# Ego-J/I2VSGG

Measured on AMD Instinct MI355X. Metric: frames/sec (600x1000, 32 ROI/frame), higher is better.
Workload: dtype f32; 1 GPU; BASELINE.json configs[1]: cfgs/res101.yml, SGG_emb fwd+bwd+SGD, 2 frames/GPU 600x1000, 32 boxes + 32 pairs/frame, ResNet-101 C4; frames_per_gpu=2, global_frames=2, hip_graph=True, parallelism=dp1 (frames sharded, RCCL all-reduce of vrd grads)

## Files before the change

### i2vsgg_amd/_lib.py

```python
import ctypes as C
import os

import torch

_HERE = os.path.dirname(os.path.abspath(__file__))
LIB_PATH = os.path.join(_HERE, "libi2vsgg_hip.so")

LAYOUT_NHWC, LAYOUT_NCHW = 0, 1
EPI_RELU, EPI_RESIDUAL, EPI_SCALE, EPI_BIAS, EPI_ZEROED = 1, 2, 4, 8, 16

_p, _i, _f, _z, _l = C.c_void_p, C.c_int32, C.c_float, C.c_size_t, C.c_int64

SIGNATURES = {
    "i2v_version": (_i, []),
    "i2v_last_error": (C.c_char_p, []),
    "i2v_build_flags": (_i, []),
    "i2v_stream_create": (_i, [_i, _i, C.POINTER(C.c_void_p)]),
    "i2v_stream_destroy": (_i, [_p]),
    "i2v_roi_align_fwd": (_i, [_p, _i, _i, _i, _i, _i, _p, _i, _i, _i, _f, _i, _p, _i, _p]),
    "i2v_roi_align_bwd": (_i, [_p, _i, _p, _i, _i, _i, _f, _i, _p, _i, _i, _i, _i, _i, _p]),
    "i2v_roi_align_bwd_gather_workspace_bytes": (_z, [_i, _i, _i, _i, _i]),
    "i2v_roi_align_bwd_gather": (_i, [_p, _p, _i, _i, _i, _f, _i, _p, _i, _i, _i, _i, _p, _z, _p]),
    "i2v_roi_align_sampled_fwd": (_i, [_p, _i, _i, _i, _i, _i, _p, _i, _i, _i, _f, _i, _p, _i, _p]),
    "i2v_roi_align_sampled_bwd": (_i, [_p, _i, _p, _i, _i, _i, _f, _i, _p, _i, _i, _i, _i, _i, _p]),
    "i2v_roi_pool_fwd": (_i, [_p, _i, _i, _i, _i, _i, _p, _i, _i, _i, _f, _p, _p, _i, _p]),
    "i2v_roi_pool_fwd_geom": (_i, [_p, _i, _i, _p, _l, _p, _i, _i, _i, _f, _p, _p, _i, _p]),
    "i2v_roi_pool_bwd": (_i, [_p, _p, _i, _p, _i, _i, _i, _p, _i, _i, _i, _i, _i, _p]),
    "i2v_nms_workspace_bytes": (_z, [_i, _i]),
    "i2v_nms_sorted": (_i, [_p, _i, _i, _f, _i, _p, _p, _p, _z, _p]),
    "i2v_rpn_proposal_workspace_bytes": (_z, [_i, _i, _i, _i, _i]),
    "i2v_rpn_proposal": (_i, [_p, _i, _p, _p, _p, _i, _i, _i, _i, _i, _i, _i, _f, _p, _p, _p, _p, _z, _p]),
    "i2v_rpn_decode": (_i, [_p, _i, _p, _p, _p, _i, _i, _i, _i, _i, _p, _p, _p]),
    "i2v_sort_desc_workspace_bytes": (_z, [_i, _i]),
    "i2v_sort_desc": (_i, [_p, _i, _i, _p, _p, _z, _p]),
    "i2v_bbox_overlaps": (_i, [_p, _i, _i, _i, _p, _i, _i, _i, _p, _p, _p, _p]),
    "i2v_conv_fwd": (_i, [_p, _p, _p, _p, _p, _p, _i, _i, _i, _i, _i, _i, _i, _i, _i, _i, _p, _z, _p]),
    "i2v_conv_fwd_splits": (_i, [_i, _i, _i, _i, _i, _i, _i, _i, _i, _z]),
    "i2v_conv_split_workspace_bytes": (_z, [_i, _i, _i, _i, _i, _i, _i, _i, _i]),
    "i2v_conv_fwd_plan": (_i, [_i, _i, _i, _i, _i, _i, _i, _i, _i, _i, _i, _z, _p, _i]),
    "i2v_conv_wgrad_plan": (_i, [_i, _i, _i, _i, _i, _i, _i, _i, _i, _i, _i, _i, _i, _i, _z, _p, _i]),
    "i2v_set_tuning": (_i, [_i, _i]),
    "i2v_get_tuning": (_i, [_i]),
    "i2v_gemm_nt_batched": (_i, [_p, _p, _p, _i, _i, _i, _i, _l, _l, _l, _p, _z, _p]),
    "i2v_winograd_filter": (_i, [_p, _p, _i, _i, _p]),
    "i2v_conv3x3_winograd_workspace_bytes": (_z, [_i, _i, _i, _i, _i]),
    "i2v_conv3x3_winograd_fwd": (_i, [_p, _p, _p, _p, _p, _i, _i, _i, _i, _i, _i, _p, _z, _p]),
    "i2v_winograd4_filter": (_i, [_p, _p, _i, _i, _p]),
    "i2v_winograd4_filter_dgrad": (_i, [_p, _p, _i, _i, _p]),
    "i2v_conv3x3_winograd4_workspace_bytes": (_z, [_i, _i, _i, _i, _i]),
    "i2v_conv3x3_winograd4_fwd": (_i, [_p, _p, _p, _p, _p, _i, _i, _i, _i, _i, _i, _p, _z, _p]),
    "i2v_conv_set_tile": (_i, [_i]),
    "i2v_conv_debug_clock": (_i, [_p]),
    "i2v_debug_clock_stamp": (_i, [_p, _p]),
    "i2v_conv_dgrad_workspace_bytes": (_z, [_i, _i, _i, _i]),
    "i2v_conv_dgrad": (_i, [_p, _p, _p, _i, _i, _i, _i, _i, _i, _i, _i, _i, _p, _z, _p, _z, _p]),
    "i2v_conv_wgrad_workspace_bytes": (_z, [_i, _i, _i, _i, _i, _i, _i, _i, _i]),
    "i2v_conv_wgrad": (_i, [_p, _p, _p, _i, _i, _i, _i, _i, _i, _i, _i, _i, _f, _p, _z, _p]),
    "i2v_conv_dgrad_fused": (_i, [_p, _p, _p, _p, _p, _p, _p, _i, _i, _i, _i, _i, _i, _i, _i, _i, _p, _z, _p, _z, _p]),
    "i2v_conv_wgrad_scaled": (_i, [_p, _p, _p, _p, _i, _i, _i, _i, _i, _i, _i, _i, _i, _f, _p, _z, _p]),
    "i2v_ordered_fallbacks": (_i, [_i]),
    "i2v_conv3x3_winograd4_dgrad": (_i, [_p, _p, _p, _p, _p, _i, _i, _i, _i, _i, _p, _z, _p]),
    "i2v_conv3x3_winograd4_wgrad_workspace_bytes": (_z, [_i, _i, _i, _i, _i]),
    "i2v_conv3x3_winograd4_wgrad": (_i, [_p, _p, _p, _p, _i, _i, _i, _i, _i, _f, _p, _z, _p]),
    "i2v_gemm_tn_batched": (_i, [_p, _p, _p, _i, _i, _i, _i, _l, _l, _l, _p]),
    "i2v_gemm_tn_batched_acc": (_i, [_p, _p, _p, _i, _i, _i, _i, _l, _l, _l, _p]),
    "i2v_conv3x3_winograd4_v_bytes": (_z, [_i, _i, _i, _i]),
    "i2v_conv3x3_winograd4_fwd_keep": (_i, [_p, _p, _p, _p, _p, _p, _i, _i, _i, _i, _i, _i, _p, _z, _p]),
    "i2v_conv3x3_winograd4_wgrad_v": (_i, [_p, _p, _p, _p, _i, _i, _i, _i, _i, _f, _p, _z, _p]),
    "i2v_conv_wgrad_sgd": (_i, [_p, _p, _p, _p, _i, _i, _i, _i, _i, _i, _i, _i, _i, _f, _f, _f, _p]),
    "i2v_epilogue_bwd": (_i, [_p, _p, _p, _p, _p, _p, _l, _i, _i, _p, _p, _z, _p]),
    "i2v_maxpool3x3s2_fwd": (_i, [_p, _p, _p, _i, _i, _i, _i, _p]),
    "i2v_sgd_momentum": (_i, [_p, _p, _p, _l, _f, _f, _f, _p]),
    "i2v_sgd_momentum_multi": (_i, [_p, _p, _p, _p, _p, _p, _i, _f, _p]),
    "i2v_adam_step": (_i, [_p, _p]),
    "i2v_adam_multi": (_i, [_p, _p, _p, _p, _p, _p, _p, _i, C.c_double, C.c_double, C.c_double, _p, _p]),
    "i2v_dstyle_pool_fwd": (_i, [_p, _p, _p, _l, _i, _i, _i, _p]),
    "i2v_dstyle_pool_bwd": (_i, [_p, _p, _p, _p, _p, _l, _i, _i, _i, _p]),
    "i2v_dstyle_fused_workspace_bytes": (_z, [_l, _i, _i, _i]),
    "i2v_dstyle_fused_fwd": (_i, [_p, _p, _p, _p, _p, _p, _p, _p, _l, _i, _i, _i, _i, _p, _z, _p]),
    "i2v_relation_topk_workspace_bytes": (_z, [_i, _i]),
    "i2v_relation_topk": (_i, [_p, _p, _p, _p, _i, _i, _i, _p, _p, _p, _p, _z, _p]),
    "i2v_video_associate_workspace_bytes": (_z, [_i, _i, _i]),
    "i2v_video_associate": (_i, [_p, _p, _p, _p, _p, _p, _i, _i, _i, _i, _p, _p, _p, _p, _p, _p, _z, _p]),
    "i2v_video_viou_match_workspace_bytes": (_z, [_i, _i]),
    "i2v_video_viou_match": (_i, [_p, _p, _p, _p, _p, _p, _i, _i, _i, _l, _i, _i, C.c_double, _p, _p, _p, _p, _z, _p]),
    "i2v_seqnms_workspace_bytes": (_z, [_i, _i, _i]),
    "i2v_seqnms": (_i, [_p, _p, _p, _p, _p, _i, _i, _i, C.c_double, C.c_double, _i, _p, _p, _p, _p, _z, _p]),
    "i2v_det_eval_match_workspace_bytes": (_z, [_i]),
    "i2v_det_eval_match": (_i, [_p, _p, _p, _p, _p, _p, _p, _i, _i, _i, _i, _i, C.c_double, _p, _p, _p, _p, _z, _p]),
    "i2v_det_eval_curve_workspace_bytes": (_z, [_i]),
    "i2v_det_eval_curve": (_i, [_p, _p, _p, _p, _i, _i, _p, _p, _p, _p, _p, _p, _p, _p, _z, _p]),
    "i2v_image_prep_size": (_i, [_i, _i, _i, _p, _p, _p]),
    "i2v_image_prep": (_i, [_p, _i, _i, _i, _i, _p, _i, _p, _i, _i, _p]),
    "i2v_det_postprocess_workspace_bytes": (_z, [_i, _i]),
    "i2v_det_postprocess": (_i, [_p, _p, _p, _i, _p, _p, _f, _f, _f, _i, _i, _f, _f, _i, _p, _p, _p, _z, _p]),
    "i2v_det_postprocess_info": (_i, [_p, _p, _p, _i, _p, _p, _p, _i, _i, _f, _f, _i, _p, _p, _p, _z, _p]),
    "i2v_l2norm_rows_fwd": (_i, [_p, _p, _p, _i, _i, _f, _p]),
    "i2v_l2norm_rows_bwd": (_i, [_p, _p, _p, _p, _i, _i, _f, _p]),
    "i2v_bce_rows_fwd": (_i, [_p, _p, _p, _p, _i, _i, _p]),
    "i2v_bce_rows_bwd": (_i, [_p, _p, _p, _p, _p, _i, _i, _p]),
    "i2v_half_mse_fwd": (_i, [_p, _l, _f, _p, _p]),
    "i2v_half_mse_bwd": (_i, [_p, _l, _f, _p, _p, _p]),
    "i2v_smooth_l1_fwd": (_i, [_p, _p, _p, _p, _l, _i, _i, _f, _p, _p]),
    "i2v_smooth_l1_bwd": (_i, [_p, _p, _p, _p, _l, _i, _i, _f, _p, _p, _p]),
    "i2v_bbox_transform": (_i, [_p, _i, _p, _i, _p, _i, _i, _p, _p, _p]),
    "i2v_signed_sqrt_fwd": (_i, [_p, _p, _l, _p]),
    "i2v_signed_sqrt_bwd": (_i, [_p, _p, _p, _l, _p]),
    "i2v_pair_gather_fwd": (_i, [_p, _p, _p, _p, _i, _i, _i, _p]),
    "i2v_pair_gather_bwd": (_i, [_p, _p, _p, _p, _i, _i, _i, _p]),
    "i2v_dpixel_fwd": (_i, [_p, _p, _p, _p, _p, _p, _p, _p, _i, _i, _p]),
    "i2v_dpixel_bwd_workspace_bytes": (_z, []),
    "i2v_dpixel_bwd": (_i, [_p, _p, _p, _p, _p, _p, _p, _p, _p, _p, _p, _p, _i, _i, _f, _p, _z, _p]),
}


class I2VError(RuntimeError):
    pass


def _load():
    if not os.path.exists(LIB_PATH):
        raise ImportError(
            "i2vsgg_amd: %s not found. Build it with `python -c 'import __graft_entry__ as g; g.build()'` "
# ... 48 lines not shown
```

### i2vsgg_amd/conv_route.py

```python
from collections import namedtuple

EPI_RELU, EPI_RESIDUAL, EPI_SCALE, EPI_BIAS = 1, 2, 4, 8

DIRECT = "direct"
WINOGRAD = "winograd"
AS_WGRAD = "as_wgrad"
WINOGRAD_X = "winograd_x"
WINOGRAD_V = "winograd_v"
NONE = "none"
ARENA, FRESH = "arena", "fresh"

Switches = namedtuple("Switches", "winograd_train winograd_wgrad winograd_keep_v winograd_train_min_c linear_dgrad_as_wgrad "
                                  "small_gw_bytes")
Route = namedtuple("Route", "fwd keep_v dgrad dgrad_pad transposed_g wgrad flags as_linear")


def whole_filter_as_linear(in_shape, w_shape, pad, has_res):
    _, _, H, W = in_shape
    _, _, KH, KW = w_shape
    return pad == 0 and KH == H and KW == W and (KH > 1 or KW > 1) and not has_res


def epilogue_flags(scale, shift, res, relu):
    return (EPI_SCALE if scale else EPI_BIAS if shift else 0) | (EPI_RESIDUAL if res else 0) | (EPI_RELU if relu else 0)


def plan_dgrad(in_shape, w_shape, stride, pad, sw):
    B, Cin, H, W = in_shape
    Cout, _, KH, KW = w_shape
    if ((H, W, KH, KW, stride, pad) == (1, 1, 1, 1, 1, 0) and B <= Cin
            and (Cout * Cin >= sw.linear_dgrad_as_wgrad or Cout % 4 != 0)):
        return AS_WGRAD, 0
    return DIRECT, (-Cout) % 4


def plan_conv(in_shape, w_shape, stride, pad, sw, scale=False, shift=False, res=False, relu=False, winograd_ok=False,
              needs_x=False, needs_w=False, needs_bias=False, in_block=False):
    as_linear = whole_filter_as_linear(in_shape, w_shape, pad, res)
    if as_linear:
        (B, Cin, H, W), Cout = in_shape, w_shape[0]
        in_shape, w_shape = (B, H * W * Cin, 1, 1), (Cout, H * W * Cin, 1, 1)
    B, Cin, H, W = in_shape
    Cout, _, KH, KW = w_shape
    flags = epilogue_flags(scale, shift, res, relu)
    eligible = (sw.winograd_train and (KH, KW, stride, pad) == (3, 3, 1, 1) and Cin >= sw.winograd_train_min_c
                and Cout >= sw.winograd_train_min_c and Cin % 4 == 0)
    wgrad_ok = eligible and sw.winograd_wgrad and Cout % 4 == 0
    if in_block:
        fwd = WINOGRAD if eligible else DIRECT
        keep_v = bool(eligible and sw.winograd_keep_v and wgrad_ok)
        wgrad = NONE if not needs_w else (WINOGRAD_V if keep_v else WINOGRAD_X) if wgrad_ok else DIRECT
        return Route(fwd, keep_v, fwd, 0, False, wgrad, flags, as_linear)
    fwd_wino = bool(winograd_ok and eligible and (needs_x or needs_w) and not res)
    keep_v = bool(fwd_wino and sw.winograd_keep_v and needs_w and wgrad_ok)
    dgrad_wino = fwd_wino or wgrad_ok
    plain, plain_pad = plan_dgrad(in_shape, w_shape, stride, pad, sw)
    dgrad = NONE if not needs_x else WINOGRAD if dgrad_wino else plain
    transposed_g = bool(dgrad == AS_WGRAD and (relu or scale or needs_bias))
    wgrad = NONE if not needs_w else (WINOGRAD_V if keep_v else WINOGRAD_X) if wgrad_ok else DIRECT
    return Route(WINOGRAD if fwd_wino else DIRECT, keep_v, dgrad, plain_pad if dgrad == DIRECT else 0, transposed_g, wgrad,
                 flags, as_linear)


def wgrad_placement(n_elems, pixels, has_arena, sw):
    return ARENA if has_arena and n_elems * 4 <= sw.small_gw_bytes and pixels > 224 else FRESH
```

### i2vsgg_amd/csrc/api.cpp

```cpp
#include <hip/hip_runtime.h>
#include <stdarg.h>
#include <stdio.h>
#include "../../include/i2vsgg_hip.h"

static thread_local char g_err[512] = "";

void i2v_set_error(const char* fmt, ...) {
    va_list ap;
    va_start(ap, fmt);
    vsnprintf(g_err, sizeof(g_err), fmt, ap);
    va_end(ap);
}

extern "C" int32_t i2v_version(void) { return 104; }
extern "C" const char* i2v_last_error(void) { return g_err; }

int g_i2v_tuning[I2V_TUNE_COUNT] = {
     -1,  2,  -1,  256,  2,
     1,  1,  128,  0,  1,
     1,  0,  2,  4,  1,
     0,  0,  0,  0,  1,
     0,  1000000,  1,  1,  1,  2,
     1,
};

extern "C" int32_t i2v_build_flags(void) {
    return 0;
}

extern "C" int32_t i2v_set_tuning(int32_t key, int32_t value) {
    if (key < 0 || key >= I2V_TUNE_COUNT) {
        i2v_set_error("set_tuning: unknown key %d", key);
        return I2V_ERR_ARG;
    }
    const bool retired = key == I2V_TUNE_CONV_SPEC ? value > 0
                       : (key == I2V_TUNE_FC_FOLD || key == I2V_TUNE_GEMM_X3 || key == I2V_TUNE_GEMM_PERSIST ||
                          key == I2V_TUNE_WGRAD_PRIO || key == I2V_TUNE_STAGGER) ? value != 0 : false;
    if (retired) {
        i2v_set_error("set_tuning: key %d belonged to an experiment kernel that is no longer in the library", key);
        return I2V_ERR_UNSUPPORTED;
    }
    g_i2v_tuning[key] = value;
    return I2V_OK;
}


extern "C" int32_t i2v_get_tuning(int32_t key) {
    return (key < 0 || key >= I2V_TUNE_COUNT) ? I2V_ERR_ARG : g_i2v_tuning[key];
}

extern "C" int32_t i2v_stream_create(int32_t device, int32_t priority, void** stream) {
    if (!stream) {
        i2v_set_error("stream_create: null output");
        return I2V_ERR_ARG;
    }
    int prev = -1, n = 0;
    if (hipGetDeviceCount(&n) != hipSuccess || device < 0 || device >= n) {
        i2v_set_error("stream_create: no device %d (%d visible)", device, n);
        return I2V_ERR_ARG;
    }
    hipStream_t s = nullptr;
    hipError_t e = hipGetDevice(&prev);
    if (e == hipSuccess && prev != device) e = hipSetDevice(device);
    if (e == hipSuccess) {
        int lo = 0, hi = 0;
        e = hipDeviceGetStreamPriorityRange(&lo, &hi);
        if (e == hipSuccess) {
// ... 23 lines not shown
```

### i2vsgg_amd/csrc/heads.hip

```cpp
#include "common.h"

namespace {

constexpr int POOL_ROWS = 64;

__global__ void dstyle_pool_fwd_kernel(const float* __restrict__ x1, const float* __restrict__ x2,
                                       float* __restrict__ z, long long rows, int dim, int rank) {
    extern __shared__ float part[];
    const int N = dim * rank;
    const int img = blockIdx.y;
    const long long r0 = (long long)blockIdx.x * POOL_ROWS;
    const long long r1 = r0 + POOL_ROWS < rows ? r0 + POOL_ROWS : rows;
    const float* a = x1 + ((long long)img * rows) * N + threadIdx.x * 4;
    const float* b = x2 + ((long long)img * rows) * N + threadIdx.x * 4;
    float4 s = make_float4(0.f, 0.f, 0.f, 0.f);
    for (long long r = r0; r < r1; ++r) {
        float4 u = *(const float4*)(a + r * N), v = *(const float4*)(b + r * N);
        s.x += u.x * v.x; s.y += u.y * v.y; s.z += u.z * v.z; s.w += u.w * v.w;
    }
    *(float4*)&part[threadIdx.x * 4] = s;
    __syncthreads();
    for (int d = threadIdx.x; d < dim; d += blockDim.x) {
        float t = 0.f;
        for (int r = 0; r < rank; ++r) t += part[d * rank + r];
// ... 243 lines not shown
    const float gl = gloss[0];
    for (long long i = blockIdx.x * (long long)blockDim.x + threadIdx.x; i < n; i += (long long)gridDim.x * blockDim.x) {
        const int row = (int)(i / cols);
        const float zz = z[i];
        const float sg = 1.f / (1.f + expf(-zz));
        gz[i] = (sg - t[i]) * (w[row] / (float)cols) * gl;
    }
}

__global__ void __launch_bounds__(256)
pair_gather_fwd_kernel(const float* __restrict__ obj, const long long* __restrict__ ixs, const long long* __restrict__ ixo,
                       float* __restrict__ out, int n_pairs, int n_box, int E) {
    const int p = blockIdx.x * 4 + (threadIdx.x >> 6), lane = threadIdx.x & 63;
    if (p >= n_pairs) return;
    const long long s = ixs[p], o = ixo[p];
    const bool sok = s >= 0 && s < n_box, ook = o >= 0 && o < n_box;
    for (int c = lane; c < E; c += 64) {
        out[(long long)p * 2 * E + c] = sok ? obj[s * E + c] : 0.f;
        out[(long long)p * 2 * E + E + c] = ook ? obj[o * E + c] : 0.f;
    }
}
__global__ void __launch_bounds__(256)
pair_gather_bwd_kernel(const float* __restrict__ g, const long long* __restrict__ ixs, const long long* __restrict__ ixo,
                       float* __restrict__ gobj, int n_pairs, int n_box, int E) {
    const int b = blockIdx.x * 4 + (threadIdx.x >> 6), lane = threadIdx.x & 63;
    if (b >= n_box) return;
    for (int c0 = 0; c0 < E; c0 += 64 * 4) {
        float a[4] = {0.f, 0.f, 0.f, 0.f};
        for (int p = 0; p < n_pairs; ++p) {
            const bool hs = ixs[p] == b, ho = ixo[p] == b;
            if (!hs && !ho) continue;
#pragma unroll
            for (int u = 0; u < 4; ++u) {
                const int c = c0 + u * 64 + lane;
                if (c < E) a[u] += (hs ? g[(long long)p * 2 * E + c] : 0.f) + (ho ? g[(long long)p * 2 * E + E + c] : 0.f);
            }
        }
#pragma unroll
        for (int u = 0; u < 4; ++u) {
            const int c = c0 + u * 64 + lane;
            if (c < E) gobj[(long long)b * E + c] = a[u];
        }
    }
}

__global__ void dp_transpose_kernel(const float* __restrict__ w, float* __restrict__ wt, int N, int K) {
    const long long total = (long long)N * K;
    for (long long i = blockIdx.x * (long long)blockDim.x + threadIdx.x; i < total; i += (long long)gridDim.x * blockDim.x) {
        const int n = (int)(i % N), k = (int)(i / N);
        wt[i] = w[(long long)n * K + k];
    }
}

}

extern "C" int32_t i2v_dstyle_pool_fwd(const float* x1, const float* x2, float* z, int64_t rows, int32_t n_img,
                                       int32_t dim, int32_t rank, void* stream) {
    I2V_CHECK_ARG(x1 && x2 && z && rows > 0 && n_img > 0 && dim > 0 && rank > 0, "dstyle_pool_fwd: bad argument");
    const int N = dim * rank;
    I2V_CHECK_ARG(N % 4 == 0 && N / 4 <= 1024, "dstyle_pool_fwd: dim*rank must be a multiple of 4 and <= 4096");
    hipStream_t st = (hipStream_t)stream;
    hipMemsetAsync(z, 0, sizeof(float) * (size_t)n_img * dim, st);
    dstyle_pool_fwd_kernel<<<dim3(i2v_cdiv(rows, POOL_ROWS), n_img), N / 4, (size_t)N * 4, st>>>(x1, x2, z, rows, dim,
                                                                                                   rank);
    I2V_CHECK_LAUNCH("dstyle_pool_fwd");
    return I2V_OK;
}

extern "C" int32_t i2v_dstyle_pool_bwd(const float* gz, const float* x1, const float* x2, float* g1, float* g2,
                                       int64_t rows, int32_t n_img, int32_t dim, int32_t rank, void* stream) {
    I2V_CHECK_ARG(gz && x1 && x2 && g1 && g2 && rows > 0 && n_img > 0 && dim > 0 && rank > 0,
                  "dstyle_pool_bwd: bad argument");
    const long long total = (long long)n_img * rows * dim * rank;
    dstyle_pool_bwd_kernel<<<(int)fmin((double)i2v_cdiv(total, 256), 16384.0), 256, 0, (hipStream_t)stream>>>(
        gz, x1, x2, g1, g2, rows, n_img, dim, rank);
    I2V_CHECK_LAUNCH("dstyle_pool_bwd");
    return I2V_OK;
}

extern "C" int32_t i2v_dpixel_fwd(const float* x, const float* w1, const float* w2, const float* w3, float* h1, float* h2,
                                  float* d, float* feat, int32_t M, int32_t pix_per_roi, void* stream) {
    I2V_CHECK_ARG(x && w1 && w2 && w3 && h1 && h2 && d && M >= 0 && pix_per_roi > 0, "dpixel_fwd: bad argument");
    I2V_CHECK_ARG(!feat || M % pix_per_roi == 0, "dpixel_fwd: M must be a whole number of ROIs when feat is requested");
    if (M == 0) return I2V_OK;
    hipStream_t st = (hipStream_t)stream;
    static bool attr = [] {
        (void)hipFuncSetAttribute((const void*)dpixel_fwd_kernel, hipFuncAttributeMaxDynamicSharedMemorySize, DP_LDS_FLOATS * 4);
        (void)hipFuncSetAttribute((const void*)dpixel_bwd_kernel, hipFuncAttributeMaxDynamicSharedMemorySize, DP_LDS_FLOATS * 4);
        return true;
    }();
    (void)attr;
    if (feat) hipMemsetAsync(feat, 0, sizeof(float) * (size_t)(M / pix_per_roi) * 128, st);
    dpixel_fwd_kernel<<<i2v_cdiv(M, DP_ROWS), DP_THREADS, DP_LDS_FLOATS * 4, st>>>(x, w1, w2, w3, h1, h2, d, feat, M,
                                                                                 pix_per_roi);
    I2V_CHECK_LAUNCH("dpixel_fwd");
    return I2V_OK;
}

extern "C" size_t i2v_dpixel_bwd_workspace_bytes(void) { return sizeof(float) * (size_t)(1024 * 512 + 512 * 128); }

extern "C" int32_t i2v_dpixel_bwd(const float* gd, const float* gfeat, const float* d, const float* h1, const float* h2,
                                  const float* w1, const float* w2, const float* w3, float* g3, float* gh2, float* gh1,
                                  float* gx, int32_t M, int32_t pix_per_roi, float lambda, void* workspace,
                                  size_t workspace_bytes, void* stream) {
    I2V_CHECK_ARG((gd || gfeat) && d && h1 && h2 && w1 && w2 && w3 && g3 && gh2 && gh1 && gx && M >= 0 && pix_per_roi > 0,
                  "dpixel_bwd: bad argument");
// ... 205 lines not shown
```

### i2vsgg_amd/launch.py

```python
import ctypes
import os

import torch

from . import _lib
from ._lib import check, lib, ptr, stream


class ZeroArena:

    def __init__(self, nbytes, device):
        self.buf = torch.zeros(max(int(nbytes), 1024) // 4, dtype=torch.float32, device=device)
        self.off = self.used = self.wanted = 0

    def reset(self):
        n = self.buf.numel() if torch.cuda.is_current_stream_capturing() else self.used
        if n:
            self.buf[:n].zero_()
        self.off = self.wanted = 0

    def take(self, B, C, H, W):
        n = B * C * H * W
        n_al = (n + 63) // 64 * 64
        self.wanted += n_al
        if self.off + n_al > self.buf.numel():
            return None
        t = self.buf[self.off:self.off + n].view(B, H, W, C).permute(0, 3, 1, 2)
        self.off += n_al
        self.used = max(self.used, self.off)
        return t

    def take_flat(self, n):
        n_al = (n + 63) // 64 * 64
        self.wanted += n_al
        if self.off + n_al > self.buf.numel():
            return None
        t = self.buf[self.off:self.off + n]
        self.off += n_al
        self.used = max(self.used, self.off)
        return t


class SplitWorkspace:
    BYTES = (48 << 20) + 4096

    def __init__(self, device, nbytes=None):
        self.buf = torch.zeros(int(nbytes or self.BYTES), dtype=torch.uint8, device=device)


_TUNE_SPLIT_ATOMICS = 4
ORDERED_SUMS = os.environ.get("I2V_ORDERED_SUMS", "1") != "0"
_ENTERED = []
_DEFAULTS = {}


class LaunchContext:

    def __init__(self, device, arena=True, ordered=False, lazy_split=False):
        self.device = torch.device(device)
        self.arena = ZeroArena(1024, self.device) if arena else None
        self.split = None if lazy_split else SplitWorkspace(self.device)
        self.scratch = {}
        self.ordered = bool(ordered)
        self.borrows_arena, self._side = False, None

    def fit(self):
        a = self.arena
        if a is not None and a.wanted * 4 > a.buf.numel() * 4:
            self.arena = ZeroArena(int(a.wanted * 4 * 1.05) + 4096, self.device)

    def side(self):
        if self._side is None:
            self._side = LaunchContext(self.device, arena=False, lazy_split=True)
            self._side.borrows_arena = True
        self._side.arena = self.arena
        return self._side

    def __enter__(self):
        self._tune = None
        if self.ordered and ORDERED_SUMS:
            self._tune = lib.i2v_get_tuning(_TUNE_SPLIT_ATOMICS)
            if self._tune == 2:
                lib.i2v_set_tuning(_TUNE_SPLIT_ATOMICS, 0)
        if self.arena is not None and not self.borrows_arena:
            self.arena.reset()
        _ENTERED.append(self)
        return self

    def __exit__(self, *exc):
        _ENTERED.pop()
        if self._tune == 2:
            lib.i2v_set_tuning(_TUNE_SPLIT_ATOMICS, 2)
        return False


def current(device=None):
    if _ENTERED:
        return _ENTERED[-1]
    index = device.index if device is not None and device.index is not None else torch.cuda.current_device()
    key = (index, stream())
    ctx = _DEFAULTS.get(key)
    if ctx is None:
        ctx = _DEFAULTS[key] = LaunchContext(torch.device("cuda", index), arena=False, lazy_split=True)
    return ctx


def arena():
    return current().arena


def split_buffer(device):
    ctx = current(device)
    if ctx.split is None:
        ctx.split = SplitWorkspace(ctx.device)
    return ctx.split.buf


def split_args(device=None):
    t = split_buffer(device)
    return ptr(t), t.numel()


def workspace(nbytes, device, tag="default"):
    cache = current(device).scratch
    buf = cache.get(tag)
    if buf is None or buf.numel() < nbytes:
        buf = torch.empty(max(int(nbytes), 256), dtype=torch.uint8, device=device)
        cache[tag] = buf
    return buf


_ROLE_STREAMS = {}
STREAM_REQUESTS = []


def role_stream(device, role, priority=0):
    dev = torch.device(device)
    index = dev.index if dev.index is not None else torch.cuda.current_device()
    key = (index, role, int(priority))
    if len(STREAM_REQUESTS) < 4096:
        STREAM_REQUESTS.append(role)
    st = _ROLE_STREAMS.get(key)
    if st is None:
        torch.cuda.init()
        out = ctypes.c_void_p()
        check(lib.i2v_stream_create(index, int(priority), ctypes.byref(out)), "i2v_stream_create")
        taken = {t.cuda_stream for t in _ROLE_STREAMS.values()}
        if not out.value or out.value in taken:
            raise _lib.I2VError("role_stream: the runtime handed out stream handle %r twice" % out.value)
        st = _ROLE_STREAMS[key] = torch.cuda.ExternalStream(out.value, device=torch.device("cuda", index))
    return st


def stream_table():
    return {k: v.cuda_stream for k, v in _ROLE_STREAMS.items()}


# ... 77 lines not shown
```

### i2vsgg_amd/ops.py

```python

import ctypes

import numpy as np
import torch

from . import _lib, conv_route, launch
from ._lib import EPI_RELU, EPI_RESIDUAL, EPI_SCALE, EPI_ZEROED, LAYOUT_NCHW, LAYOUT_NHWC, check, lib, ptr, stream
from .conv_route import ARENA, AS_WGRAD, DIRECT, WINOGRAD, WINOGRAD_V

_CL = torch.channels_last


def _need_cuda(*ts):
    for t in ts:
        if t is not None and not t.is_cuda:
            raise _lib.I2VError("i2vsgg_amd ops run on the GPU only (got a %s tensor); there is no CPU fallback"
                                % t.device.type)


def as_nhwc(x):
    if x.dim() != 4:
        raise ValueError("expected a 4-D (B,C,H,W) tensor")
    if x.dtype != torch.float32:
        x = x.float()
# ... 380 lines not shown
    if conv_route.wgrad_placement(n, B * g.shape[2] * g.shape[3], arena is not None, _switches()) == ARENA:
        flat = arena.take_flat(n)
        if flat is not None:
            gw, beta = flat.view(Cout, KH, KW, Cin).permute(0, 3, 1, 2), 1.0
    if gw is None:
        gw = torch.empty(w_shape, device=x.device, dtype=torch.float32, memory_format=_CL)
    if route != DIRECT:
        ws = launch.workspace(lib.i2v_conv3x3_winograd4_wgrad_workspace_bytes(B, H, W, Cin, Cout), x.device, "winograd_wgrad")
        with _Timed(2.0 * B * H * W * Cout * 9 * Cin, tag, "N%d K%d M%d (3x3 winograd F4)" % (Cout, 9 * Cin, B * H * W),
                    4 * (x.numel() + g.numel() + gw.numel())):
            if route == WINOGRAD_V:
                check(lib.i2v_conv3x3_winograd4_wgrad_v(ptr(v), ptr(g), ptr(row_scale), ptr(gw), B, H, W, Cin, Cout, beta, ptr(ws),
                                                        ws.numel(), stream()), "conv3x3_winograd4_wgrad_v")
            else:
                check(lib.i2v_conv3x3_winograd4_wgrad(ptr(x), ptr(g), ptr(row_scale), ptr(gw), B, H, W, Cin, Cout, beta, ptr(ws),
                                                      ws.numel(), stream()), "conv3x3_winograd4_wgrad")
        return gw
    with _Timed(2.0 * B * g.shape[2] * g.shape[3] * Cout * KH * KW * Cin, tag,
                "N%d K%d M%d" % (Cout, KH * KW * Cin, B * g.shape[2] * g.shape[3]) + (" (wgrad form)" if tag != "wgrad" else ""),
                4 * (x.numel() + g.numel() + gw.numel())):
        sws = launch.split_buffer(x.device)
        if row_scale is not None:
            check(lib.i2v_conv_wgrad_scaled(ptr(x), ptr(g), ptr(row_scale), ptr(gw), B, H, W, Cin, Cout, KH, KW, stride, pad,
                                            beta, ptr(sws), sws.numel(), stream()), "conv_wgrad_scaled")
        else:
            check(lib.i2v_conv_wgrad(ptr(x), ptr(g), ptr(gw), B, H, W, Cin, Cout, KH, KW, stride, pad, beta,
                                     ptr(sws), sws.numel(), stream()), "conv_wgrad")
    return gw


FUSED_SGD = {}


class FusedEntry(tuple):

    def __new__(cls, m, lr, momentum, wd, owner=None):
        self = super().__new__(cls, (m, lr, momentum, wd))
        self.owner = owner
        return self


def _conv_wgrad_sgd_raw(x, g, w, cfg, stride, pad):
    m, lr, mom, wd = cfg
    B, Cin, H, W = x.shape
    Cout, _, KH, KW = w.shape
    with _Timed(2.0 * B * g.shape[2] * g.shape[3] * Cout * KH * KW * Cin, "wgrad",
                "N%d K%d M%d +sgd" % (Cout, KH * KW * Cin, B * g.shape[2] * g.shape[3]),
                4 * (x.numel() + g.numel() + 4 * w.numel())):
        rc = lib.i2v_conv_wgrad_sgd(ptr(x), ptr(g), ptr(w), ptr(m), B, H, W, Cin, Cout, KH, KW, stride, pad, float(lr),
                                    float(mom), float(wd), stream())
    return rc


class _ConvFn(torch.autograd.Function):

    @staticmethod
    def forward(ctx, x, w, scale, shift, res, stride, pad, relu, wino_ok=False):
        _need_cuda(x, w)
        x = as_nhwc(x)
        w = as_nhwc(w)
        if res is not None:
            res = as_nhwc(res)
        need = ctx.needs_input_grad
        route = _plan(x.shape, w.shape, stride, pad, scale=scale is not None, shift=shift is not None, res=res is not None,
                      relu=relu, winograd_ok=wino_ok, needs_x=need[0], needs_w=need[1],
                      needs_bias=need[3] and shift is not None and scale is None)
        v = None
        if route.fwd == WINOGRAD:
            y, v = _winograd_fwd(x, winograd_filter(w.detach(), 4), scale, shift, relu, keep_v=route.keep_v)
        else:
            y = _conv_fwd_raw(x, w, scale, shift, res, stride, pad, route.flags)
        ctx.route = route
        ctx.cfg = (stride, pad, relu, scale is not None, shift is not None, res is not None)
        ctx.save_for_backward(x, w, scale, y if relu else None, v)
        return y

    @staticmethod
    def backward(ctx, gy):
        x, w, scale, y, v = ctx.saved_tensors
        stride, pad, relu, has_scale, has_shift, has_res = ctx.cfg
        route = ctx.route
        gy = as_nhwc(gy)
        M, N = gy.shape[0] * gy.shape[2] * gy.shape[3], gy.shape[1]
        gres = g_t = None
        need_bias = ctx.needs_input_grad[3] and has_shift and not has_scale
        need_res = has_res and ctx.needs_input_grad[4]
        gbias = None
        if need_bias:
            arena = launch.arena()
            gbias = arena.take_flat(N) if arena is not None else None
            if gbias is None:
                gbias = torch.zeros((N,), device=gy.device, dtype=torch.float32)

        if relu or has_scale or need_bias:
            want_pre = need_res and (relu or has_scale)
            want_g = has_scale or relu
            g = torch.empty_like(gy) if want_g else None
            gpre = torch.empty_like(gy) if (want_pre and has_scale) else None
            if route.transposed_g:
                g_t = torch.empty((N, M, 1, 1), device=gy.device, dtype=torch.float32)
            check(lib.i2v_epilogue_bwd(ptr(gy), ptr(y), ptr(scale) if has_scale else None, ptr(g), ptr(gpre), ptr(gbias),
                                       M, N, int(relu), ptr(g_t), *launch.split_args(), stream()), "epilogue_bwd")
            if g is None:
                g = gy
            if need_res:
                gres = gpre if gpre is not None else g
        else:
            g = gy
            gres = gy if need_res else None
        gx = None
        if ctx.needs_input_grad[0]:
            if route.dgrad == WINOGRAD:
                gx, _ = _winograd_fwd(g, winograd_filter_dgrad(w), tag="dgrad")
            else:
                gx = _conv_dgrad_raw(g, w, x.shape, stride, pad, (route.dgrad, route.dgrad_pad), g_t)
        gw = None
        if ctx.needs_input_grad[1]:
            fused = FUSED_SGD.get(w.data_ptr())
            if fused is None or _conv_wgrad_sgd_raw(x, g, w, fused, stride, pad) != 0:
                gw = _conv_wgrad_raw(x, g, w.shape, stride, pad, route=route.wgrad, v=v)
        return gx, gw, None, gbias, gres, None, None, None, None


def _winograd_dgrad_fused(g, U, out_scale, mask):
    B, Cout, H, W = g.shape
    Cin = U.shape[1]
    gx = torch.empty((B, Cin, H, W), device=g.device, dtype=torch.float32, memory_format=_CL)
    ws = launch.workspace(lib.i2v_conv3x3_winograd4_workspace_bytes(B, H, W, Cout, Cin), g.device, "winograd")
    T = B * ((H + 3) // 4) * ((W + 3) // 4)
    with _Timed(2.0 * B * H * W * Cout * 9 * Cin, "dgrad",
                "M%d N%d K%d (3x3 winograd F4) gemmMB=%.2f +epi" % (B * H * W, Cin, 9 * Cout, 4e-6 * 36 * (T * Cout + Cout * Cin + T * Cin)),
                4 * (g.numel() + 9 * Cout * Cin + 2 * gx.numel())):
        check(lib.i2v_conv3x3_winograd4_dgrad(ptr(g), ptr(U), ptr(out_scale), ptr(mask), ptr(gx), B, H, W, Cout, Cin, ptr(ws),
                                              ws.numel(), stream()), "conv3x3_winograd4_dgrad")
# ... 721 lines not shown
```

### i2vsgg_amd/train.py

```python
import numpy as np
import torch

from . import _lib, launch, ops, parallel
from . import synthetic as syn
from .graphs import CapturedStep, replay_graph, _REPLAY_STREAMS
from .model.utils.config import cfg
from .optim import FusedSGD, FusedAdam, make_optimizer, _same_memory_order
from .staging import (_Slot, _place_u8, parse_u8_meta, place_frames, step_uploader, synthetic_sgg_batch,
                      sgg_head_inputs, _rasterize_host)


class _FrameSet:

    def __init__(self, key, device, n_ctx, arena):
        n, h, w = key
        self.key = key
        self.im = torch.zeros((n, 4, h, w), device=device).contiguous(memory_format=torch.channels_last)
        self.ctx = [launch.LaunchContext(device, arena=arena) for _ in range(n_ctx)]
        self.fh = self.fw = None
        self.graph = None
        self.fitted = False
        self.tick = 0
        self.ctx_front = launch.LaunchContext(device, arena=arena)
        self.ctx_back = launch.LaunchContext(device, arena=arena)
# ... 24 lines not shown

    def call(self):
        head = None if self.bubble else self.cur
        if head is not None:
            self.last_trained = head
        self.cur, self.mid = self.mid, self.inp
        return head


class SGGEmbStep(CapturedStep):

    def __init__(self, net, n_frames, vrd_lr=1e-4, seed=1, device="cuda:0", h=600, w=1000, n_boxes=32, n_pairs=32,
                 use_graph=True, fuse_sgd=True, zero_arena=True, overlap=None, max_graphs=16, trace_rows=0, stage_synthetic=True,
                 optimizer="sgd", bb_split=None):
        import os
        self.net, self.dev, self.n_frames = net, torch.device(device), n_frames
        if not (net.vrd.use_obj_visual and net.vrd.spatial_type == 2):
            raise ValueError("SGGEmbStep packs the inputs of the reference's default relation head (use_obj_visual=True, "
                             "spatial_type=2: what every reference script runs); the other vrd variants run through "
                             "vrd.forward / forward_device")
        self.world = parallel.world_size()
        self.geom = (h, w, n_boxes, n_pairs)
        self.tp = parallel.exchange_enabled() and os.environ.get("I2V_TP_FC6", "1") != "0" and \
            net.vrd.fc6.fc.weight.shape[0] % max(self.world, 1) == 0
        if self.tp and net.vrd.tp is None:
            net.vrd.enable_fc6_tp(parallel.rank(), self.world)
        self.opt = make_optimizer(optimizer, [(n, p) for n, p in net.named_parameters() if n.startswith("vrd.")], vrd_lr)
        self.fused = self.opt.fuse_wgrad() if fuse_sgd else []
        self.loss = torch.zeros((), device=self.dev)
        self._seed = torch.full((), 1.0 / max(self.world, 1), device=self.dev)
        self.graph_error = None
        self.use_graph = use_graph
        if overlap is None:
            overlap = os.environ.get("I2V_OVERLAP", "1") != "0"
        self.overlap = bool(overlap) and use_graph
        self._pipelined = False
        self._graphs_on = False
        self.zero_arena = zero_arena
        mode = bb_split if bb_split is not None else os.environ.get("I2V_BB_SPLIT", "stage")
        mode = {"1": "frame", "0": "none", "2": "stage"}.get(str(mode), str(mode))
        if mode not in ("stage", "frame", "none"):
            raise ValueError("SGGEmbStep: bb_split must be 'stage', 'frame' or 'none', got %r" % (mode,))
        self.stage_split = mode == "stage" and use_graph
        self.bb_split = mode == "frame" and use_graph and n_frames > 1
        n3 = len(net.RCNN_base[6])
        self.cut = max(1, min(int(os.environ.get("I2V_STAGE_CUT", "6")), max(n3 // 3, 1), n3 - 1))
        self._frame_streams = [launch.role_stream(self.dev, ("frame", f)) for f in range(max(n_frames, 2))] \
            if (self.bb_split or self.stage_split) else []
        self._pipe, self.n_bubbles = _StagePipeline(), 0
        self._mid_key = None
        self.mid_next_flat = self.mid_cur_flat = None
        self.mid_slot = None
        self._side = None
        self.ctx_head = launch.LaunchContext(self.dev, arena=zero_arena, ordered=True)
        self.ctx_bb = launch.LaunchContext(self.dev, arena=zero_arena)
        self.shapes, self.max_graphs, self._tick, self._pool = {}, int(max_graphs), 0, None
        self.cap_boxes, self.cap_pairs = n_frames * n_boxes, n_frames * n_pairs
        self.cap_cells = 0
        self.fmap_flat = self.fmap_head_flat = None
        self.cur = self.inp = None
        self._staged = None
        self._fmap_key = None
        self.primed = False
        self.trace = torch.zeros((trace_rows, len(self.TRACE_COLS)), device=self.dev, dtype=torch.float64) if trace_rows else None
        self._trace_i = torch.zeros((1,), device=self.dev, dtype=torch.long)
        if stage_synthetic:
            self.reseed(seed)

    @property
    def lag(self):
        return (2 if self.stage_split else 1) if self._pipelined else 0

    @property
    def bubble(self):
        return bool(self._pipelined and self.stage_split and self._pipe.bubble)

    @property
    def graph(self):
        fs = self.shapes.get(self._staged)
        return (fs.graph or None) if fs is not None else None

    @property
    def im(self):
        return self.shapes[self._staged].im

    @property
    def fmap(self):
        fs = self.shapes[self._fmap_key]
        n, c = fs.key[0], self._channels
        return self.fmap_flat[:n * fs.fh * fs.fw * c].view(n, fs.fh, fs.fw, c).permute(0, 3, 1, 2)

    def _layout(self, nb, npair):
        f32, i64 = torch.float32, torch.long
        return {"rois": ((nb + npair, 5), f32), "labels": ((npair, self.net.vrd.n_rel), f32), "ix12": ((2 * npair,), i64),
                "masks": ((npair, 4, 32, 32), f32), "wrow": ((npair,), f32), "extent": ((2,), torch.int32)}

    def _synthetic(self, seed):
        h, w, n_boxes, n_pairs = self.geom
        head = self.net.vrd
        im, info, annos = synthetic_sgg_batch(seed, self.n_frames, n_boxes, n_pairs, head.n_rel, head.n_obj, h, w)
        head.source_gt_rels = annos
        self.paths = sorted(annos, key=lambda s: int(s[1:]))
        fields = sgg_head_inputs([annos[p] for p in self.paths], info, head.n_rel)
        im4 = torch.zeros((im.shape[0], 4) + tuple(im.shape[2:]), device=self.dev).contiguous(memory_format=torch.channels_last)
        im4[:, :3] = torch.from_numpy(im).to(self.dev)
        return im4, info, fields

# ... 831 lines not shown
```

### include/i2vsgg_hip.h

```cpp
#ifndef I2VSGG_HIP_H
#define I2VSGG_HIP_H

#include <stdint.h>
#include <stddef.h>

#ifdef __cplusplus
extern "C" {
#endif

#define I2V_OK               0
#define I2V_ERR_ARG         -1
#define I2V_ERR_LAUNCH      -2
#define I2V_ERR_WORKSPACE   -3
#define I2V_ERR_UNSUPPORTED -4

#define I2V_LAYOUT_NHWC 0
#define I2V_LAYOUT_NCHW 1

#define I2V_EPI_RELU      1
#define I2V_EPI_RESIDUAL  2
#define I2V_EPI_SCALE     4
#define I2V_EPI_BIAS      8
#define I2V_EPI_ZEROED   16
#define I2V_EPI_MASK     32
// ... 173 lines not shown
int32_t i2v_conv3x3_winograd4_dgrad(const float* gy, const float* U, const float* out_scale, const float* mask,
                                    float* gx, int32_t B, int32_t H, int32_t W, int32_t Cout, int32_t Cin,
                                    void* workspace, size_t workspace_bytes, void* stream);
size_t  i2v_conv3x3_winograd4_wgrad_workspace_bytes(int32_t B, int32_t H, int32_t W, int32_t Cin, int32_t Cout);
int32_t i2v_conv3x3_winograd4_wgrad(const float* x, const float* gy, const float* row_scale, float* gw,
                                    int32_t B, int32_t H, int32_t W, int32_t Cin, int32_t Cout, float beta,
                                    void* workspace, size_t workspace_bytes, void* stream);
size_t  i2v_conv3x3_winograd4_v_bytes(int32_t B, int32_t H, int32_t W, int32_t Cin);
int32_t i2v_conv3x3_winograd4_fwd_keep(const float* x, const float* U, const float* scale, const float* shift,
                                       float* y, float* v_out, int32_t B, int32_t H, int32_t W, int32_t Cin,
                                       int32_t Cout, int32_t relu, void* workspace, size_t workspace_bytes, void* stream);
int32_t i2v_conv3x3_winograd4_wgrad_v(const float* v, const float* gy, const float* row_scale, float* gw,
                                      int32_t B, int32_t H, int32_t W, int32_t Cin, int32_t Cout, float beta,
                                      void* workspace, size_t workspace_bytes, void* stream);
int32_t i2v_gemm_tn_batched(const float* x, const float* gy, float* gw, int32_t M, int32_t N, int32_t K,
                            int32_t nbatch, long long stride_x, long long stride_gy, long long stride_gw, void* stream);
int32_t i2v_gemm_tn_batched_acc(const float* x, const float* gy, float* gw, int32_t M, int32_t N, int32_t K,
                            int32_t nbatch, long long stride_x, long long stride_gy, long long stride_gw, void* stream);
size_t  i2v_conv_dgrad_workspace_bytes(int32_t Cin, int32_t Cout, int32_t KH, int32_t KW);
int32_t i2v_conv_dgrad(const float* gy, const float* w, float* gx, int32_t B, int32_t H, int32_t W,
                       int32_t Cin, int32_t Cout, int32_t KH, int32_t KW, int32_t stride, int32_t pad,
                       void* workspace, size_t workspace_bytes, void* split_workspace, size_t split_workspace_bytes,
                       void* stream);
size_t  i2v_conv_wgrad_workspace_bytes(int32_t B, int32_t H, int32_t W, int32_t Cin, int32_t Cout,
                                       int32_t KH, int32_t KW, int32_t stride, int32_t pad);
int32_t i2v_conv_wgrad(const float* x, const float* gy, float* gw, int32_t B, int32_t H, int32_t W,
                       int32_t Cin, int32_t Cout, int32_t KH, int32_t KW, int32_t stride, int32_t pad,
                       float beta, void* workspace, size_t workspace_bytes, void* stream);

int32_t i2v_gemm_nt_batched(const float* a, const float* b, float* c, int32_t M, int32_t N, int32_t K, int32_t nbatch,
                            int64_t stride_a, int64_t stride_b, int64_t stride_c,
                            void* split_workspace, size_t split_workspace_bytes, void* stream);

int32_t i2v_winograd_filter(const float* w, float* U, int32_t Cout, int32_t Cin, void* stream);
size_t  i2v_conv3x3_winograd_workspace_bytes(int32_t B, int32_t H, int32_t W, int32_t Cin, int32_t Cout);
int32_t i2v_conv3x3_winograd_fwd(const float* x, const float* U, const float* scale, const float* shift, float* y,
                                 int32_t B, int32_t H, int32_t W, int32_t Cin, int32_t Cout, int32_t relu,
                                 void* workspace, size_t workspace_bytes, void* stream);

int32_t i2v_winograd4_filter(const float* w, float* U, int32_t Cout, int32_t Cin, void* stream);
int32_t i2v_winograd4_filter_dgrad(const float* w, float* U, int32_t Cout, int32_t Cin, void* stream);
size_t  i2v_conv3x3_winograd4_workspace_bytes(int32_t B, int32_t H, int32_t W, int32_t Cin, int32_t Cout);
int32_t i2v_conv3x3_winograd4_fwd(const float* x, const float* U, const float* scale, const float* shift, float* y,
                                  int32_t B, int32_t H, int32_t W, int32_t Cin, int32_t Cout, int32_t relu,
                                  void* workspace, size_t workspace_bytes, void* stream);

int32_t i2v_conv_wgrad_sgd(const float* x, const float* gy, float* w, float* m, int32_t B, int32_t H, int32_t W,
                           int32_t Cin, int32_t Cout, int32_t KH, int32_t KW, int32_t stride, int32_t pad,
                           float lr, float momentum, float weight_decay, void* stream);

int32_t i2v_epilogue_bwd(const float* gy, const float* y, const float* scale, float* g, float* gpre, float* gbias,
                         int64_t M, int32_t N, int32_t relu, float* g_t, void* split_ws, size_t split_ws_bytes, void* stream);

int32_t i2v_maxpool3x3s2_fwd(const float* x, float* y, int32_t* argmax, int32_t B, int32_t H, int32_t W, int32_t C,
                             void* stream);

int32_t i2v_dstyle_pool_fwd(const float* x1, const float* x2, float* z, int64_t rows, int32_t n_img,
                            int32_t dim, int32_t rank, void* stream);
int32_t i2v_dstyle_pool_bwd(const float* gz, const float* x1, const float* x2, float* g1, float* g2,
                            int64_t rows, int32_t n_img, int32_t dim, int32_t rank, void* stream);
size_t  i2v_dstyle_fused_workspace_bytes(int64_t rows, int32_t n_img, int32_t dim, int32_t rank);
int32_t i2v_dstyle_fused_fwd(const float* x, const float* w1, const float* b1, const float* w2, const float* b2,
                             float* z, float* x1, float* x2, int64_t rows, int32_t n_img, int32_t k, int32_t dim,
                             int32_t rank, void* workspace, size_t workspace_bytes, void* stream);

int32_t i2v_l2norm_rows_fwd(const float* x, float* y, float* inv_norm, int32_t rows, int32_t cols, float eps, void* stream);
int32_t i2v_l2norm_rows_bwd(const float* g, const float* y, const float* inv_norm, float* gx, int32_t rows, int32_t cols,
                            float eps, void* stream);
int32_t i2v_bce_rows_fwd(const float* z, const float* t, const float* w, float* loss, int32_t rows, int32_t cols,
                         void* stream);
int32_t i2v_bce_rows_bwd(const float* z, const float* t, const float* w, const float* gloss, float* gz, int32_t rows,
                         int32_t cols, void* stream);

int32_t i2v_pair_gather_fwd(const float* obj, const int64_t* ixs, const int64_t* ixo, float* out, int32_t n_pairs,
                            int32_t n_box, int32_t emb, void* stream);
int32_t i2v_pair_gather_bwd(const float* g, const int64_t* ixs, const int64_t* ixo, float* gobj, int32_t n_pairs,
                            int32_t n_box, int32_t emb, void* stream);

int32_t i2v_half_mse_fwd(const float* d, int64_t n, float target, float* out, void* stream);
int32_t i2v_half_mse_bwd(const float* d, int64_t n, float target, const float* gout, float* gd, void* stream);
int32_t i2v_smooth_l1_fwd(const float* pred, const float* tgt, const float* inw, const float* outw, int64_t n, int32_t per_weight,
                          int32_t rows, float sigma, float* out, void* stream);
int32_t i2v_smooth_l1_bwd(const float* pred, const float* tgt, const float* inw, const float* outw, int64_t n, int32_t per_weight,
                          int32_t rows, float sigma, const float* gout, float* gpred, void* stream);
int32_t i2v_bbox_transform(const float* ex, int32_t ex_batched, const float* gt, int32_t gt_stride, float* out, int32_t B, int32_t N,
                           const float* means4, const float* stds4, void* stream);
int32_t i2v_signed_sqrt_fwd(const float* z, float* y, int64_t n, void* stream);
int32_t i2v_signed_sqrt_bwd(const float* z, const float* g, float* gz, int64_t n, void* stream);

int32_t i2v_dpixel_fwd(const float* x, const float* w1, const float* w2, const float* w3, float* h1, float* h2,
                       float* d, float* feat, int32_t M, int32_t pix_per_roi, void* stream);
size_t  i2v_dpixel_bwd_workspace_bytes(void);
int32_t i2v_dpixel_bwd(const float* gd, const float* gfeat, const float* d, const float* h1, const float* h2,
                       const float* w1, const float* w2, const float* w3, float* g3, float* gh2, float* gh1,
                       float* gx, int32_t M, int32_t pix_per_roi, float lambda, void* workspace,
                       size_t workspace_bytes, void* stream);

int32_t i2v_sgd_momentum(float* p, const float* g, float* m, int64_t n, float lr, float momentum,
                         float weight_decay, void* stream);
int32_t i2v_sgd_momentum_multi(float* const* p, const float* const* g, float* const* m, const int64_t* n,
                               const float* lr, const float* weight_decay, int32_t count, float momentum,
                               void* stream);

int32_t i2v_adam_step(int32_t* step_counter, void* stream);
int32_t i2v_adam_multi(float* const* p, const float* const* g, float* const* m, float* const* v, const int64_t* n,
                       const double* lr, const float* weight_decay, int32_t count, double beta1, double beta2, double eps,
// ... 7 lines not shown
```

Measured before the change: 509.7 frames/s.

## Fuse small linear-layer backward into one MFMA kernel for head layers

Adds a single HIP kernel that computes weight gradient, input gradient, bias gradient and the ReLU mask for small fully connected layers (at most 128 rows, weights up to 2^21). It uses f32 MFMA tiles, with weight-gradient and input-gradient blocks sharing one launch. The head LaunchContext routes eligible 1x1/whole-filter convs to it, replacing the separate epilogue, dgrad and wgrad launches. The goal is to cut launch count and intermediate traffic in the ROI/relation heads, at the cost of a fixed tiling that may underuse the GPU for some shapes.

```diff
diff --git a/i2vsgg_amd/_lib.py b/i2vsgg_amd/_lib.py
--- a/i2vsgg_amd/_lib.py
+++ b/i2vsgg_amd/_lib.py
@@ -69,6 +69,7 @@
     "i2v_conv3x3_winograd4_wgrad_v": (_i, [_p, _p, _p, _p, _i, _i, _i, _i, _i, _f, _p, _z, _p]),
     "i2v_conv_wgrad_sgd": (_i, [_p, _p, _p, _p, _i, _i, _i, _i, _i, _i, _i, _i, _i, _f, _f, _f, _p]),
     "i2v_epilogue_bwd": (_i, [_p, _p, _p, _p, _p, _p, _l, _i, _i, _p, _p, _z, _p]),
+    "i2v_linear_bwd_small": (_i, [_p, _p, _p, _p, _p, _p, _p, _i, _i, _i, _l, _l, _p]),
     "i2v_maxpool3x3s2_fwd": (_i, [_p, _p, _p, _i, _i, _i, _i, _p]),
     "i2v_sgd_momentum": (_i, [_p, _p, _p, _l, _f, _f, _f, _p]),
     "i2v_sgd_momentum_multi": (_i, [_p, _p, _p, _p, _p, _p, _i, _f, _p]),
diff --git a/i2vsgg_amd/conv_route.py b/i2vsgg_amd/conv_route.py
--- a/i2vsgg_amd/conv_route.py
+++ b/i2vsgg_amd/conv_route.py
@@ -34,6 +34,21 @@
     return DIRECT, (-Cout) % 4
 
 
+SMALL_LINEAR_ROWS, SMALL_LINEAR_WEIGHTS = 128, 1 << 21
+
+
+def small_linear_bwd(in_shape, w_shape, stride, pad, scale=False, res=False, needs_w=False, fused=False):
+    if whole_filter_as_linear(in_shape, w_shape, pad, res):
+        (B, Cin, H, W), Cout = in_shape, w_shape[0]
+        in_shape, w_shape = (B, H * W * Cin, 1, 1), (Cout, H * W * Cin, 1, 1)
+    B, Cin, H, W = in_shape
+    Cout, _, KH, KW = w_shape
+    if (H, W, KH, KW, stride, pad) != (1, 1, 1, 1, 1, 0):
+        return False
+    return bool(not scale and not res and needs_w and not fused and B <= SMALL_LINEAR_ROWS
+                and Cout * Cin <= SMALL_LINEAR_WEIGHTS and Cin % 4 == 0)
+
+
 def plan_conv(in_shape, w_shape, stride, pad, sw, scale=False, shift=False, res=False, relu=False, winograd_ok=False,
               needs_x=False, needs_w=False, needs_bias=False, in_block=False):
     as_linear = whole_filter_as_linear(in_shape, w_shape, pad, res)
diff --git a/i2vsgg_amd/csrc/api.cpp b/i2vsgg_amd/csrc/api.cpp
--- a/i2vsgg_amd/csrc/api.cpp
+++ b/i2vsgg_amd/csrc/api.cpp
@@ -12,7 +12,7 @@
     va_end(ap);
 }
 
-extern "C" int32_t i2v_version(void) { return 104; }
+extern "C" int32_t i2v_version(void) { return 105; }
 extern "C" const char* i2v_last_error(void) { return g_err; }
 
 int g_i2v_tuning[I2V_TUNE_COUNT] = {
diff --git a/i2vsgg_amd/csrc/heads.hip b/i2vsgg_amd/csrc/heads.hip
--- a/i2vsgg_amd/csrc/heads.hip
+++ b/i2vsgg_amd/csrc/heads.hip
@@ -319,6 +319,125 @@
     }
 }
 
+constexpr int LB_T = 64;
+constexpr int LB_TM = 32;
+constexpr int LB_LD = 80;
+
+__device__ inline float lb_g(const float* __restrict__ gy, const float* __restrict__ y, long long ldg, long long ldy,
+                             int m, int n, int M, int N) {
+    if (m >= M || n >= N) return 0.f;
+    const float v = gy[m * ldg + n];
+    if (y) return y[m * ldy + n] > 0.f ? v : 0.f;
+    return v;
+}
+
+__device__ inline void lb_stage_rows(const float* __restrict__ src, int r0, int rows, int k0, int K, float* dst) {
+#pragma unroll
+    for (int it = 0; it < 4; ++it) {
+        const int rr = (threadIdx.x >> 4) + 16 * it, c = (threadIdx.x & 15) * 4;
+        float4 v = make_float4(0.f, 0.f, 0.f, 0.f);
+        if (r0 + rr < rows && k0 + c < K) v = *(const float4*)(src + (long long)(r0 + rr) * K + k0 + c);
+        *(float4*)&dst[rr * LB_LD + c] = v;
+    }
+}
+
+template <int NT>
+__device__ inline void lb_mma(const float* As, const float* Bs, int acol, int bcol, f32x4 (&acc)[NT]) {
+    const int lane = threadIdx.x & 63, fr = lane & 15, fg = lane >> 4;
+#pragma unroll
+    for (int s = 0; s < LB_T / 4; ++s) {
+        const float a = As[(4 * s + fg) * LB_LD + acol + fr];
+#pragma unroll
+        for (int t = 0; t < NT; ++t) {
+            const float b = Bs[(4 * s + fg) * LB_LD + bcol + 16 * t + fr];
+            acc[t] = __builtin_amdgcn_mfma_f32_16x16x4f32(a, b, acc[t], 0, 0, 0);
+        }
+    }
+}
+
+__global__ void __launch_bounds__(256)
+linear_bwd_small_kernel(const float* __restrict__ x, const float* __restrict__ w, const float* __restrict__ gy,
+                        const float* __restrict__ y, float* __restrict__ gw, float* __restrict__ gx,
+                        float* __restrict__ gbias, int M, int N, int K, long long ldg, long long ldy, int k_tiles,
+                        int gw_blocks) {
+    __shared__ float As[LB_T * LB_LD], Bs[LB_T * LB_LD];
+    const int tid = threadIdx.x, wave = tid >> 6, lane = tid & 63, fr = lane & 15, fg = lane >> 4;
+    int blk = blockIdx.x;
+    if (blk < gw_blocks) {
+        const int k0 = (blk % k_tiles) * LB_T, n0 = (blk / k_tiles) * LB_T;
+        const bool bias = gbias && k0 == 0 && tid < LB_T;
+        f32x4 acc[4];
+#pragma unroll
+        for (int t = 0; t < 4; ++t) acc[t] = (f32x4){0.f, 0.f, 0.f, 0.f};
+        float bs[4] = {0.f, 0.f, 0.f, 0.f};
+        for (int m0 = 0; m0 < M; m0 += LB_T) {
+#pragma unroll
+            for (int it = 0; it < 16; ++it) {
+                const int mm = wave + 4 * it;
+                As[mm * LB_LD + lane] = lb_g(gy, y, ldg, ldy, m0 + mm, n0 + lane, M, N);
+            }
+            lb_stage_rows(x, m0, M, k0, K, Bs);
+            __syncthreads();
+            if (bias)
+                for (int mm = 0; mm < LB_T; mm += 4) {
+                    bs[0] += As[mm * LB_LD + tid]; bs[1] += As[(mm + 1) * LB_LD + tid];
+                    bs[2] += As[(mm + 2) * LB_LD + tid]; bs[3] += As[(mm + 3) * LB_LD + tid];
+                }
+            lb_mma<4>(As, Bs, 16 * wave, 0, acc);
+            __syncthreads();
+        }
+#pragma unroll
+        for (int t = 0; t < 4; ++t)
+#pragma unroll
+            for (int r = 0; r < 4; ++r) {
+                const int n = n0 + 16 * wave + 4 * fg + r, k = k0 + 16 * t + fr;
+                if (n < N && k < K) gw[(long long)n * K + k] = acc[t][r];
+            }
+        if (bias && n0 + tid < N) gbias[n0 + tid] = (bs[0] + bs[1]) + (bs[2] + bs[3]);
+        return;
+    }
+    blk -= gw_blocks;
+    const int k0 = (blk % k_tiles) * LB_T, m0 = (blk / k_tiles) * LB_TM;
+    f32x4 acc[2];
+    acc[0] = acc[1] = (f32x4){0.f, 0.f, 0.f, 0.f};
+    for (int n0 = 0; n0 < N; n0 += LB_T) {
+#pragma unroll
+        for (int it = 0; it < 8; ++it) {
+            const int idx = it * 256 + tid;
+            const int nn = (idx >> 7) * 4 + (idx & 3), mm = (idx >> 2) & 31;
+            As[nn * LB_LD + mm] = lb_g(gy, y, ldg, ldy, m0 + mm, n0 + nn, M, N);
+        }
+        lb_stage_rows(w, n0, N, k0, K, Bs);
+        __syncthreads();
+        lb_mma<2>(As, Bs, 16 * (wave & 1), 32 * (wave >> 1), acc);
+        __syncthreads();
+    }
+#pragma unroll
+    for (int t = 0; t < 2; ++t)
+#pragma unroll
+        for (int r = 0; r < 4; ++r) {
+            const int m = m0 + 16 * (wave & 1) + 4 * fg + r, k = k0 + 32 * (wave >> 1) + 16 * t + fr;
+            if (m < M && k < K) gx[(long long)m * K + k] = acc[t][r];
+        }
+}
+
+}
+
+extern "C" int32_t i2v_linear_bwd_small(const float* x, const float* w, const float* gy, const float* y, float* gw, float* gx,
+                                        float* gbias, int32_t M, int32_t N, int32_t K, int64_t ldg, int64_t ldy,
+                                        void* stream) {
+    I2V_CHECK_ARG(x && w && gy && gw && M >= 0 && N >= 1 && K >= 4, "linear_bwd_small: bad argument");
+    I2V_CHECK_ARG(M <= 128 && K % 4 == 0 && (long long)N * K <= (1ll << 21),
+                  "linear_bwd_small: M <= 128, K %% 4 == 0 and N * K <= 2^21 (got M %d, N %d, K %d)", M, N, K);
+    I2V_CHECK_ARG(ldg >= N && (!y || ldy >= N), "linear_bwd_small: a row stride below N");
+    I2V_CHECK_ARG(((uintptr_t)x | (uintptr_t)w) % 16 == 0, "linear_bwd_small: x and w must be 16-byte aligned");
+    const int k_tiles = i2v_cdiv(K, LB_T);
+    const int gw_blocks = i2v_cdiv(N, LB_T) * k_tiles;
+    const int gx_blocks = gx ? i2v_cdiv(M, LB_TM) * k_tiles : 0;
+    linear_bwd_small_kernel<<<gw_blocks + gx_blocks, 256, 0, (hipStream_t)stream>>>(x, w, gy, y, gw, gx, gbias, M, N, K, ldg,
+                                                                                   ldy, k_tiles, gw_blocks);
+    I2V_CHECK_LAUNCH("linear_bwd_small");
+    return I2V_OK;
 }
 
 extern "C" int32_t i2v_dstyle_pool_fwd(const float* x1, const float* x2, float* z, int64_t rows, int32_t n_img,
diff --git a/i2vsgg_amd/launch.py b/i2vsgg_amd/launch.py
--- a/i2vsgg_amd/launch.py
+++ b/i2vsgg_amd/launch.py
@@ -56,8 +56,9 @@
 
 class LaunchContext:
 
-    def __init__(self, device, arena=True, ordered=False, lazy_split=False):
+    def __init__(self, device, arena=True, ordered=False, lazy_split=False, small_linear_bwd=False):
         self.device = torch.device(device)
+        self.small_linear_bwd = bool(small_linear_bwd)
         self.arena = ZeroArena(1024, self.device) if arena else None
         self.split = None if lazy_split else SplitWorkspace(self.device)
         self.scratch = {}
@@ -103,6 +104,10 @@
     if ctx is None:
         ctx = _DEFAULTS[key] = LaunchContext(torch.device("cuda", index), arena=False, lazy_split=True)
     return ctx
+
+
+def small_linear_bwd():
+    return bool(_ENTERED) and _ENTERED[-1].small_linear_bwd
 
 
 def arena():
diff --git a/i2vsgg_amd/ops.py b/i2vsgg_amd/ops.py
--- a/i2vsgg_amd/ops.py
+++ b/i2vsgg_amd/ops.py
@@ -456,6 +456,31 @@
     return rc
 
 
+LINEAR_BWD_SMALL = True
+
+
+def _linear_bwd_small(gy, x, w, y, need_x, need_bias):
+    M, K = x.shape[0], x.shape[1]
+    N = w.shape[0]
+    if gy.dtype != torch.float32 or (N > 1 and gy.stride(1) != 1) or (M > 1 and gy.stride(0) < N):
+        gy = as_nhwc(gy)
+    ldg = gy.stride(0) if M > 1 else N
+    ldy = N
+    if y is not None:
+        if (N > 1 and y.stride(1) != 1) or (M > 1 and y.stride(0) < N):
+            raise ValueError("linear backward: the saved output is not row-major")
+        ldy = y.stride(0) if M > 1 else N
+    dev = x.device
+    gw = torch.empty(w.shape, device=dev, dtype=torch.float32, memory_format=_CL)
+    gx = torch.empty(x.shape, device=dev, dtype=torch.float32, memory_format=_CL) if need_x else None
+    gbias = torch.empty((N,), device=dev, dtype=torch.float32) if need_bias else None
+    with _Timed(2.0 * M * N * K * (2 if need_x else 1), "linear_bwd", "M%d N%d K%d" % (M, N, K),
+                4 * (x.numel() + M * N + w.numel() * (2 if need_x else 1) + (x.numel() if need_x else 0))):
+        check(lib.i2v_linear_bwd_small(ptr(x), ptr(w), ptr(gy), ptr(y), ptr(gw), ptr(gx), ptr(gbias), M, N, K, ldg, ldy,
+                                       stream()), "linear_bwd_small")
+    return gx, gw, gbias
+
+
 class _ConvFn(torch.autograd.Function):
 
     @staticmethod
@@ -484,6 +509,12 @@
         x, w, scale, y, v = ctx.saved_tensors
         stride, pad, relu, has_scale, has_shift, has_res = ctx.cfg
         route = ctx.route
+        if (LINEAR_BWD_SMALL and ctx.needs_input_grad[1] and launch.small_linear_bwd()
+                and conv_route.small_linear_bwd(tuple(x.shape), tuple(w.shape), stride, pad, scale=has_scale, res=has_res,
+                                                needs_w=True, fused=w.data_ptr() in FUSED_SGD)):
+            gx, gw, gbias = _linear_bwd_small(gy, x, w, y if relu else None, ctx.needs_input_grad[0],
+                                              ctx.needs_input_grad[3] and has_shift)
+            return gx, gw, None, gbias, None, None, None, None, None
         gy = as_nhwc(gy)
         M, N = gy.shape[0] * gy.shape[2] * gy.shape[3], gy.shape[1]
         gres = g_t = None
diff --git a/i2vsgg_amd/train.py b/i2vsgg_amd/train.py
--- a/i2vsgg_amd/train.py
+++ b/i2vsgg_amd/train.py
@@ -100,7 +100,7 @@
         self.mid_next_flat = self.mid_cur_flat = None
         self.mid_slot = None
         self._side = None
-        self.ctx_head = launch.LaunchContext(self.dev, arena=zero_arena, ordered=True)
+        self.ctx_head = launch.LaunchContext(self.dev, arena=zero_arena, ordered=True, small_linear_bwd=True)
         self.ctx_bb = launch.LaunchContext(self.dev, arena=zero_arena)
         self.shapes, self.max_graphs, self._tick, self._pool = {}, int(max_graphs), 0, None
         self.cap_boxes, self.cap_pairs = n_frames * n_boxes, n_frames * n_pairs
diff --git a/include/i2vsgg_hip.h b/include/i2vsgg_hip.h
--- a/include/i2vsgg_hip.h
+++ b/include/i2vsgg_hip.h
@@ -249,6 +249,9 @@
 int32_t i2v_epilogue_bwd(const float* gy, const float* y, const float* scale, float* g, float* gpre, float* gbias,
                          int64_t M, int32_t N, int32_t relu, float* g_t, void* split_ws, size_t split_ws_bytes, void* stream);
 
+int32_t i2v_linear_bwd_small(const float* x, const float* w, const float* gy, const float* y, float* gw, float* gx,
+                             float* gbias, int32_t M, int32_t N, int32_t K, int64_t ldg, int64_t ldy, void* stream);
+
 int32_t i2v_maxpool3x3s2_fwd(const float* x, float* y, int32_t* argmax, int32_t B, int32_t H, int32_t W, int32_t C,
                              void* stream);
 
```

Result: no change. 511.5 frames/s, median of 6 (+0.4%).
